# khimansusinha/Distributed-sorting-with-fault-tolerance

Measured on AMD Instinct MI355X. Metric: sorted keys/sec (int32, 2^30 keys), higher is better.
Workload: dtype int32; 1 GPU; C2-style single-GPU sort of 1073741824 uniform int32 keys (BASELINE metric size); tile 8192 keys, 0 merge passes; keys=1073741824, parallelism=1 GPU

## Files before the change

### distributed-sorting-with-fault-tolerance_amd/csrc/dsort_sub.h

```cpp
#pragma once
#include <hip/hip_runtime.h>
#include <stdint.h>

#include "dsort_bucket.h"

namespace dsort {
namespace sb {

constexpr int SB_T = 256;
constexpr int SB_MAXS = 1024;
constexpr int SB_SLOTB = 10;
constexpr int SB_SLOTS = 1 << SB_SLOTB;
#ifndef DSORT_SUB_TOTALS
#define DSORT_SUB_TOTALS 1
#endif
constexpr int SB_ST = 4;
template <typename T> constexpr int SB_KPT = sizeof(T) == 4 ? 16 : 8;
template <typename T> constexpr int SB_SUB = SB_T * SB_KPT<T>;
template <typename T> constexpr int SB_CH = SB_ST * SB_SUB<T>;

struct BInfo {
    uint64_t start;
    uint64_t soff;
    uint32_t len;
// ... 375 lines not shown
            aoff = off;
            v = 0;
            np = 0;
        }
        if (piece == 0 && np == 0 && v == 0) {
            ca = c + 1;
            aoff = 0;
        }
    }
    if (np) {
        f(ca, aoff, c1, v);
        ++nt;
    }
    return nt;
}
__device__ __forceinline__ uint2 tile_piece(const uint32_t *counts, int SS, uint32_t base, uint32_t c, uint32_t c0,
                                            uint32_t nch, uint32_t j0, uint32_t j1, uint32_t valid, uint32_t flags) {
    const uint32_t *pc = counts + (uint64_t)c * (SS + 1);
    const uint32_t lo = base + pc[j0] + (c == c0 ? flags >> 8 : 0u);
    return make_uint2(lo, nch == 1 ? lo + valid : base + pc[j1]);
}

#ifdef DSORT_STAMPS
__device__ unsigned long long g_sbstamps[(1u << 18) * 8];
#endif
template <bool LOCAL>
__global__ void __launch_bounds__(SB_MAXS, 8) sb_scan_kernel(const BInfo *__restrict__ bi, int SS,
                                                          const uint32_t *__restrict__ counts,
                                                          uint32_t *__restrict__ offs, int tile, int align,
                                                          uint32_t mis, uint32_t cpad, void *__restrict__ tiles,
                                                          uint32_t *__restrict__ ntiles, Ovf *__restrict__ ovf,
                                                          uint32_t *__restrict__ novf, uint32_t trec,
                                                          const Chunk *__restrict__ ch, uint2 *__restrict__ pieces,
                                                          uint32_t PS, uint32_t tcap, const uint32_t *__restrict__ stot) {
    __shared__ uint32_t wsum[SB_MAXS / 64];
    __shared__ uint32_t ss[SB_MAXS + 1];
    __shared__ uint16_t nxt[SB_MAXS];
    __shared__ uint16_t chain[SB_MAXS];
    __shared__ uint16_t tix[SB_MAXS];
    __shared__ uint32_t nchain, tbase;
#ifdef DSORT_SCAN_STAMPS
    uint64_t sc_acc[8] = {}, sc_t0 = __builtin_amdgcn_s_memtime();
#define SCST(k)                                            \
    do {                                                   \
        const uint64_t t1_ = __builtin_amdgcn_s_memtime(); \
        sc_acc[k] += t1_ - sc_t0;                          \
        sc_t0 = t1_;                                       \
    } while (0)
#else
#define SCST(k) \
    do {        \
    } while (0)
#endif
    const BInfo b = bi[blockIdx.x];
    const int j = threadIdx.x;
    const int ns = (int)b.nsub;
    const int full = tile;
    if (LOCAL) tile -= (int)(cpad * (b.c1 - b.c0));
    auto cnt = [&](uint32_t c) -> uint32_t {
        if constexpr (LOCAL) {
            const uint32_t *pc = counts + (uint64_t)c * (SS + 1);
            return pc[j + 1] - pc[j];
        } else {
            return counts[(uint64_t)c * SS + j];
        }
    };
    uint32_t tot = 0;
    if (LOCAL && stot) {
        if (j < ns) tot = stot[(uint64_t)blockIdx.x * SS + j];
    } else if constexpr (LOCAL) {
        uint32_t a = 0;
        if (j < ns) {
#ifndef DSORT_SCAN_SUM_U
#define DSORT_SCAN_SUM_U 16
#endif
#pragma unroll DSORT_SCAN_SUM_U
            for (uint32_t c = b.c0; c < b.c1; ++c) a += counts[(uint64_t)c * (SS + 1) + j + 1];
            ss[j + 1] = a;
        }
        __syncthreads();
        if (j < ns) tot = a - (j ? ss[j] : 0u);
    } else if (j < ns) {
#pragma unroll 8
        for (uint32_t c = b.c0; c < b.c1; ++c) tot += cnt(c);
    }
    uint32_t all;
// ... 491 lines not shown
```

### distributed-sorting-with-fault-tolerance_amd/csrc/dsort_wave.hip

```cpp
#include <hip/hip_runtime.h>

#include <stdint.h>

#include <algorithm>
#include <climits>
#include <ctime>
#include <sched.h>
#include <unistd.h>
#include <csignal>
#include <cstdlib>
#include <cstring>
#include <string>
#include <type_traits>
#include <vector>

#include "dsort_bucket.h"
#include "dsort_internal.h"
#include "dsort_tx.h"

#include <rocprofiler-sdk-roctx/roctx.h>
#include "dsort_part.h"
#include "dsort_sub.h"

namespace dsort {
// ... 977 lines not shown
                klo = gt.j0 > 0 ? sp[gt.j0 - 1].k : bk::Comp<T>::key_of(bs[gt.b - 1]);
                khi = gt.j1 < gt.nsub ? sp[gt.j1 - 1].k : bk::Comp<T>::key_of(bs[gt.b]);
            }
            if (jj < jh && jj + 1 < nspl) hint = sp[jj].k == sp[jj + 1].k;
            hint = __ballot(hint) != 0;
        }
        if (!late && known) {
            klo = gt.j0 > 0 ? sp[gt.j0 - 1].k : bk::Comp<T>::key_of(bs[gt.b - 1]);
            khi = gt.j1 < gt.nsub ? sp[gt.j1 - 1].k : bk::Comp<T>::key_of(bs[gt.b]);
#ifndef DSORT_ONEKEY_TILES
#define DSORT_ONEKEY_TILES 1
#endif
            if (DSORT_ONEKEY_TILES && sizeof(T) == 8 && klo == khi) {
                T *o = out + base;
                for (int i = (int)threadIdx.x; i < valid; i += (int)blockDim.x) o[i] = klo;
                return;
            }
        }
        if (!late) {
            if (jj < jh && jj + 1 < nspl) hint = sp[jj].k == sp[jj + 1].k;
            hint = __ballot(hint) != 0;
            gather_tile<T, W>(ga, pe, gt, in, s32 + 128, s32 + 96, x, threadIdx.x);
        }
    } else {
        j = toff + blockIdx.x;
        if (!load_tile<T, false, W>(in, n, tiles, ntiles, ga, j, nullptr, nullptr, x, base, valid)) return;
        if (valid == 0) return;
    }
    STAMP(1);
    if (!bin_sort_tile<T, W>(x, valid, s, cw, out + base, hint, known, klo, khi, threadIdx.x) && threadIdx.x == 0)
        fb[atomicAdd(nfb, 1u)] = j;
}

template <typename T, bool GATHER, int W>
__global__ void __launch_bounds__(64 * W, WG<T>::OCC) block_sort_w_kernel(
    const T *in, T *out, uint64_t n, const uint4 *tiles, const uint32_t *ntiles, sb::Gather ga,
    const uint32_t *fb, const uint32_t *nfb) {
    constexpr int TILE = TILE_W<W>, N = KPC<T>;
    using V = typename V16<T>::type;
    __shared__ __attribute__((aligned(16))) T s[TILE + WK];
    const int t = lane_id();
    const int w = __builtin_amdgcn_readfirstlane(threadIdx.x >> 6);
    const T c[6] = {lane_side<T>(0), lane_side<T>(1), lane_side<T>(2), lane_side<T>(3), lane_side<T>(4),
                    lane_side<T>(5)};
    const uint32_t nj = *nfb;
#pragma unroll 1
    for (uint32_t i = blockIdx.x; i < nj; i += gridDim.x) {
    if (i != blockIdx.x) __syncthreads();
    T x[R];
    uint64_t base;
    int valid;
    const uint32_t j = fb[i];
    if (!load_tile<T, GATHER, W>(in, n, tiles, ntiles, ga, j, reinterpret_cast<uint32_t *>(s) + 64,
                              reinterpret_cast<uint32_t *>(s), x, base, valid))
        return;
    if (GATHER) __syncthreads();
    sort_wave(x, c);
    {
        if (w & 1) {
            V *dst = reinterpret_cast<V *>(s + w * WK + WK - R * (t + 1));
#pragma unroll
            for (int q = 0; q < R / N; ++q) {
                T rv[N];
#pragma unroll
                for (int j = 0; j < N; ++j) rv[j] = x[R - 1 - (N * q + j)];
                dst[q] = V16<T>::make(rv);
            }
        } else {
            V *dst = reinterpret_cast<V *>(s + w * WK + t * R);
#pragma unroll
            for (int q = 0; q < R / N; ++q) dst[q] = V16<T>::make(x + N * q);
        }
    }
    __syncthreads();
    const int lo = out_lo(t);
#pragma unroll 1
    for (int r = WK; r < TILE; r <<= 1) {
        const int wpp = (2 * r) / WK;
        const int j = w / wpp, o = w % wpp;
        const int ps = j * 2 * r;
        const bool last = 2 * r == TILE;
        WinD win{ps, r, r, o * WK, 0, WK, !last && (j & 1)};
        merge_window_desc(s, win, x, c[0], c[1], c[2], c[3]);
        __syncthreads();
        if (last) {
            const int lim = valid - o * WK;
            win.cnt = lim < WK ? lim : WK;
            if (lim > 0) store_window_desc<false>(out + base, win, ps, lo, x);
        } else {
            store_window_desc<true>(s, win, ps, lo, x);
            __syncthreads();
        }
    }
    }
}

template <typename T, int LOGF, bool REG>
__global__ void __launch_bounds__(64 * WG<T>::MWAVES, WG<T>::OCC) mergew_kernel(
    const T *__restrict__ in, T *__restrict__ out, PassDesc pd, int tnom, const uint32_t *__restrict__ splits) {
    constexpr int WAVES = WG<T>::MWAVES, THREADS = 64 * WAVES, TILE = MTILE_OF<T>;
    constexpr int N = KPC<T>, LN = LKPC<T>;
    using V = typename V16<T>::type;
    constexpr int F = 1 << LOGF;
    constexpr int MAXWIN = (WAVES + F / 2 + WAVES - 1) / WAVES;
    static_assert(WAVES * MAXWIN <= 64, "window table: one lane per window");
    __shared__ __attribute__((aligned(16))) T s[TILE + WK];
    __shared__ int soff[F + 1];
    __shared__ int cpre[F + 1];
    __shared__ int4 sinfo[F];
    __shared__ int64_t sa0[F];
    __shared__ uint64_t s_out;
    __shared__ int4 wtab_a[LOGF][WAVES * MAXWIN];
    __shared__ int4 wtab_b[LOGF][WAVES * MAXWIN];
    const int t = lane_id();
    const int w = __builtin_amdgcn_readfirstlane(threadIdx.x >> 6);
    const uint64_t j = blockIdx.x;
    STAMP(0);
    RSTAMP(13);
    TileInfo ti;
    const GroupK *g = tile_info<REG>(pd, j, tnom, ti);
    if (threadIdx.x < 64) {
        const int i = t & (F - 1);
        uint64_t rs, rl;
        run_range<REG>(pd, ti, g, i, rs, rl);
        const uint32_t s0 = splits[j * F + i];
        const uint32_t s1 = ti.jr + 1 == ti.ntg ? (uint32_t)rl : splits[(j + 1) * F + i];
        const int len = (int)(s1 - s0);
// ... 156 lines not shown
    std::vector<int> out;
    const int bits = ceil_log2(runs);
    if (bits == 0) return out;
    const int cap = max_logf(opt, 4, WG<T>::MAXLOGF);
    const int P = (bits + cap - 1) / cap;
    for (int p = 0; p < P; ++p) out.push_back(bits / P + (p < bits % P ? 1 : 0));
    return out;
}

static void stage_range(const dsort_ctx *ctx, int i) {
    if (ctx->nested) return;
    switch (i) {
        case 9: roctxRangePushA("dsort:histogram"); break;
        case 11: roctxRangePushA("dsort:scatter"); break;
        case 13: roctxRangePushA("dsort:second-level"); break;
        case 7: roctxRangePushA("dsort:tile-sort"); break;
        case 10: case 12: case 14: case 8: roctxRangePop(); break;
        default: break;
    }
}
static int stage_event(dsort_ctx *ctx, hipStream_t s, bool timed, int i) {
    if (timed) stage_range(ctx, i);
    if (!timed || !ctx->ev_ok) return DSORT_OK;
    if (i == 1 || i == 7 || i == 8 || i == 13 || i == 14) i += ctx->ev_off;
    DSORT_HIP(ctx, hipEventRecord(ctx->ev[i], s));
    ctx->ev_mask |= 1u << i;
    return DSORT_OK;
}
static int tile_sort_event(dsort_ctx *ctx, hipStream_t s, bool timed, int which) {
    return stage_event(ctx, s, timed, 7 + which);
}

constexpr uint32_t kFallbackWgs = 512;
template <typename T, bool GATHER, int W>
static int tile_sort_begin(dsort_ctx *ctx, const T *in, T *out, uint64_t n, const uint4 *tiles, const uint32_t *ntiles,
                           const sb::Gather &ga, uint32_t grid, uint32_t cap, hipStream_t s) {
    int rc = ensure(ctx, &ctx->tfb, &ctx->tfb_bytes, ((size_t)cap + 1) * 4, "tile fallback list");
    if (rc) return rc;
    uint32_t *fb = static_cast<uint32_t *>(ctx->tfb), *nfb = fb + cap;
    DSORT_HIP(ctx, hipMemsetAsync(nfb, 0, 4, s));
    if (grid)
        hipLaunchKernelGGL((bin_sort_kernel<T, GATHER, W>), dim3(grid), dim3(64 * W), 0, s, in, out, n, tiles, ntiles, ga, fb,
                           nfb, 0u);
    DSORT_HIP(ctx, hipGetLastError());
    return DSORT_OK;
}
template <typename T, bool GATHER, int W>
static int tile_sort_more(dsort_ctx *ctx, const T *in, T *out, uint64_t n, const uint4 *tiles, const uint32_t *ntiles,
                          const sb::Gather &ga, uint32_t toff, uint32_t grid, uint32_t cap, hipStream_t s) {
    uint32_t *fb = static_cast<uint32_t *>(ctx->tfb), *nfb = fb + cap;
    if (grid)
        hipLaunchKernelGGL((bin_sort_kernel<T, GATHER, W>), dim3(grid), dim3(64 * W), 0, s, in, out, n, tiles, ntiles, ga, fb,
                           nfb, toff);
    DSORT_HIP(ctx, hipGetLastError());
    return DSORT_OK;
}
template <typename T, bool GATHER, int W>
static int tile_sort_end(dsort_ctx *ctx, const T *in, T *out, uint64_t n, const uint4 *tiles, const uint32_t *ntiles,
                         const sb::Gather &ga, uint32_t tiles_total, uint32_t cap, hipStream_t s) {
    const uint32_t *fb = static_cast<const uint32_t *>(ctx->tfb), *nfb = fb + cap;
    const uint32_t fgrid = tiles_total < kFallbackWgs ? tiles_total : kFallbackWgs;
    if (fgrid)
        hipLaunchKernelGGL((block_sort_w_kernel<T, GATHER, W>), dim3(fgrid), dim3(64 * W), 0, s, in, out, n, tiles, ntiles,
                           ga, fb, nfb);
    DSORT_HIP(ctx, hipGetLastError());
    return DSORT_OK;
}
template <typename T, bool GATHER, int W>
static int tile_sort_w(dsort_ctx *ctx, const T *in, T *out, uint64_t n, const uint4 *tiles, const uint32_t *ntiles,
                       const sb::Gather &ga, uint32_t grid, hipStream_t s) {
    int rc = tile_sort_begin<T, GATHER, W>(ctx, in, out, n, tiles, ntiles, ga, grid, grid, s);
    if (rc) return rc;
    return tile_sort_end<T, GATHER, W>(ctx, in, out, n, tiles, ntiles, ga, grid, grid, s);
}
template <typename T, typename F>
static int with_tile_waves(dsort_ctx *ctx, int tile, F &&f) {
    if (tile == TILE_OF<T>) return f(std::integral_constant<int, WG<T>::WAVES>{});
    if constexpr (sizeof(T) == 4)
        if (tile == TILE_W<16>) return f(std::integral_constant<int, 16>{});
    return set_err(ctx, DSORT_EINVAL, "tile sort: no kernel for this tile size");
}
template <typename T, bool GATHER>
static int tile_sort(dsort_ctx *ctx, const T *in, T *out, uint64_t n, const uint4 *tiles, const uint32_t *ntiles,
                     const sb::Gather &ga, uint32_t grid, hipStream_t s, bool timed, int tile = TILE_OF<T>) {
    int rc = tile_sort_event(ctx, s, timed, 0);
    if (rc) return rc;
    if (grid) {
        rc = with_tile_waves<T>(ctx, tile, [&](auto w) {
            return tile_sort_w<T, GATHER, decltype(w)::value>(ctx, in, out, n, tiles, ntiles, ga, grid, s);
        });
        if (rc) return rc;
    }
    return tile_sort_event(ctx, s, timed, 1);
}

template <typename T, bool REG>
static int launch_pass_w(dsort_ctx *ctx, const T *src, T *dst, const PassDesc &pd, int logf,
                         uint64_t ntiles, hipStream_t s, bool timed) {
    int rc = ensure(ctx, &ctx->splits, &ctx->splits_bytes,
                    (size_t)(ntiles + 1) * (size_t)(1 << logf) * sizeof(uint32_t), "split vectors");
    if (rc) return rc;
    uint32_t *sp = static_cast<uint32_t *>(ctx->splits);
    constexpr int TN = MTNOM_OF<T>;
    hipLaunchKernelGGL((partk_kernel<T, REG>), dim3((unsigned)ceil_div(ntiles, 4)), dim3(256), 0, s, src, pd,
                       TN, MSLACK_OF<T>, sp, ntiles);
    DSORT_HIP(ctx, hipGetLastError());
    const bool kt = timed && ctx->ev_ok && ctx->kev_used + 2 <= dsort_ctx::kMaxKev;
    if (kt) DSORT_HIP(ctx, hipEventRecord(ctx->kev[ctx->kev_used], s));
    const dim3 grid((unsigned)ntiles), block(64 * WG<T>::MWAVES);
    switch (logf) {
        case 1: hipLaunchKernelGGL((mergew_kernel<T, 1, REG>), grid, block, 0, s, src, dst, pd, TN, sp); break;
        case 2: hipLaunchKernelGGL((mergew_kernel<T, 2, REG>), grid, block, 0, s, src, dst, pd, TN, sp); break;
        case 3: hipLaunchKernelGGL((mergew_kernel<T, 3, REG>), grid, block, 0, s, src, dst, pd, TN, sp); break;
        case 4: hipLaunchKernelGGL((mergew_kernel<T, 4, REG>), grid, block, 0, s, src, dst, pd, TN, sp); break;
        case 5:
            if constexpr (WG<T>::MAXLOGF >= 5) {
                hipLaunchKernelGGL((mergew_kernel<T, 5, REG>), grid, block, 0, s, src, dst, pd, TN, sp);
                break;
            }
            return set_err(ctx, DSORT_EINVAL, "bad pass fan-in");
        default: return set_err(ctx, DSORT_EINVAL, "bad pass fan-in");
    }
    DSORT_HIP(ctx, hipGetLastError());
    if (kt) {
        DSORT_HIP(ctx, hipEventRecord(ctx->kev[ctx->kev_used + 1], s));
        ctx->kev_used += 2;
// ... 271 lines not shown
    DSORT_HIP(ctx, hipMemcpyAsync(stl, hst, B * sizeof(bk::TileRef) + 16, hipMemcpyHostToDevice, ctx->side));
    DSORT_HIP(ctx, hipMemsetAsync(num, 0, 8, ctx->side));
    if (nfill)
        DSORT_HIP(ctx, hipMemcpyAsync(a + o_fill, hf, nfill * sizeof(FillSeg<T>), hipMemcpyHostToDevice, ctx->side));
    DSORT_HIP(ctx, hipEventRecord(ctx->side_ev, ctx->side));
    DSORT_HIP(ctx, hipStreamWaitEvent(s, ctx->side_ev, 0));
    uint64_t npure = 0;
    for (int b = 0; b < B; ++b) npure += pure[b] ? hb[b + 1] - hb[b] : 0;
    ctx->stats.tile_sort_keys = n - npure;
    if (nfill) {
        const unsigned gx = (unsigned)std::min<uint64_t>(ceil_div(maxfill, 256 * FILL_U * (16 / sizeof(T))), 1024);
        hipLaunchKernelGGL(fill_segments_kernel<T>, dim3(gx, nfill), dim3(256), 0, s, d_keys,
                           reinterpret_cast<const FillSeg<T> *>(a + o_fill));
        DSORT_HIP(ctx, hipGetLastError());
    }
    for (int b = 0; b < B && !pure_done && !pm;) {
        if (!pure[b]) {
            ++b;
            continue;
        }
        int e = b;
        while (e < B && pure[e]) ++e;
        if (hb[e] > hb[b])
            DSORT_HIP(ctx, hipMemcpyAsync(d_keys + hb[b], src + hb[b], (hb[e] - hb[b]) * sizeof(T),
                                          hipMemcpyDeviceToDevice, s));
        b = e;
    }
    if (nsmp) {
        hipLaunchKernelGGL(sb_sample_kernel<T>, dim3((unsigned)B), dim3(SB_T), 0, s, src, dbi, dch, smp, cmp);
        DSORT_HIP(ctx, hipGetLastError());
        const uint4 *stl4 = reinterpret_cast<const uint4 *>(stl);
        const uint32_t *pnst = reinterpret_cast<const uint32_t *>(stl + B);
        if constexpr (sizeof(T) == 8) {
            rc = tile_sort<int64_t, false>(ctx, smp, srt, nsmp, stl4, pnst, sb::Gather{}, nst, s, false);
            if (rc) return rc;
            hipLaunchKernelGGL(sb_rank_kernel, dim3((unsigned)B), dim3(SB_T), 0, s, smp, srt, dbi, cmp);
        }
        rc = tile_sort<int64_t, false>(ctx, cmp, cmp, nsmp, stl4, pnst, sb::Gather{}, nst, s, false);
        if (rc) return rc;
        hipLaunchKernelGGL(sb_splitter_kernel<T>, dim3((unsigned)B), dim3(SB_MAXS), 0, s, cmp, smp, dbi, dch, os, SS, spl,
                           rng, sfn, stot);
        DSORT_HIP(ctx, hipGetLastError());
    } else if (stot) {
        DSORT_HIP(ctx, hipMemsetAsync(stot, 0, (size_t)B * SS * 4, s));
    }
    const uint32_t mis = (uint32_t)((reinterpret_cast<uintptr_t>(d_keys) / sizeof(T)) & (ALIGN - 1));
    uint32_t *hn = reinterpret_cast<uint32_t *>(h + h_num);
    if (local) {
        if (nch) {
            if ((rc = stage_event(ctx, s, timed, 13))) return rc;
            hipLaunchKernelGGL(sb_local_kernel<T>, dim3((unsigned)nch), dim3(SB_LT<T>), 0, s, src, dch, dbi, SS, spl, rng,
                               sfn, cnt, ctx->bk_hot, stot);
            DSORT_HIP(ctx, hipGetLastError());
            if ((rc = stage_event(ctx, s, timed, 14))) return rc;
        }
#ifndef DSORT_PIECES_SCAN_MINB
#define DSORT_PIECES_SCAN_MINB 256
#endif
        const bool pieces_in_scan = B >= DSORT_PIECES_SCAN_MINB;
        hipLaunchKernelGGL(sb_scan_kernel<true>, dim3((unsigned)B), dim3(SB_MAXS), 0, s, dbi, SS, cnt, nullptr, TILE, 1,
                           0u, (uint32_t)(2 * (ALIGN - 1)), tt, num, ovf, num + 1, (uint32_t)tmax,
                           static_cast<const Chunk *>(dch), pieces_in_scan ? pcs : nullptr, PS, (uint32_t)tcap, stot);
        DSORT_HIP(ctx, hipGetLastError());
        const Gather ga{static_cast<const GTile *>(tt), dch, dbi, cnt, pcs, PS, SS, spl, bspl, B,
                        (uint32_t)std::max<uint64_t>(tcap, 1)};
#ifndef DSORT_PIECES_EARLY
#define DSORT_PIECES_EARLY 1
#endif
        const bool pieces_early = DSORT_PIECES_EARLY && !pieces_in_scan && pcs && tcap > 0;
        if (pieces_early) {
            hipLaunchKernelGGL(sb_pieces_kernel, dim3((unsigned)ceil_div(tcap, 4)), dim3(256), 0, s,
                               static_cast<const GTile *>(tt), num, static_cast<const Chunk *>(dch), cnt, SS, pcs, PS,
                               (uint32_t)tcap);
            DSORT_HIP(ctx, hipGetLastError());
        }
        DSORT_HIP(ctx, hipMemcpyAsync(hn, num, 8, hipMemcpyDeviceToHost, s));
        DSORT_HIP(ctx, hipEventRecord(ctx->sub_ev, s));
#ifndef DSORT_TILE_EARLY
#define DSORT_TILE_EARLY 1
#endif
        const uint64_t ebound = (n - npure) / (uint64_t)TILE;
        const uint32_t early = DSORT_TILE_EARLY && (pieces_in_scan || pieces_early) && ctx->opt.kill_after_pass != 1
                                   ? (uint32_t)std::min<uint64_t>(ebound, tcap)
                                   : 0u;
        if (early) {
            if ((rc = tile_sort_event(ctx, s, timed, 0))) return rc;
            rc = with_tile_waves<T>(ctx, TILE, [&](auto w) {
                return tile_sort_begin<T, true, decltype(w)::value>(ctx, src, d_keys, n, nullptr, num, ga, early,
                                                                    (uint32_t)tcap, s);
            });
            if (rc) return rc;
        }
        if (int rc_ = sync_event(ctx, ctx->sub_ev, "tile count")) return rc_;
        const uint32_t ntiles = hn[0], novf = hn[1];
        if (ntiles > tmax || ntiles > tcap) {
            if (early)
                if (int rc_ = sync_stream(ctx, s, "early tile sort")) return rc_;
            ctx->stats.sub_scatter_fallback = 1;
            return sub_sort<T>(ctx, src, d_keys, n, hb, B, m, s, timed, false, pure, pure_done, bspl, true, pm,
                               fill_keys);
        }
        if (ntiles && !pieces_in_scan && !pieces_early) {
            hipLaunchKernelGGL(sb_pieces_kernel, dim3((unsigned)ceil_div(ntiles, 4)), dim3(256), 0, s,
                               static_cast<const GTile *>(tt), num, static_cast<const Chunk *>(dch), cnt, SS, pcs, PS,
                               (uint32_t)tcap);
            DSORT_HIP(ctx, hipGetLastError());
        }
        fault_point(ctx, s, 1);
        ctx->stats.merge_passes = 0;
        if (early) {
            rc = with_tile_waves<T>(ctx, TILE, [&](auto w) {
                constexpr int W = decltype(w)::value;
                int r = tile_sort_more<T, true, W>(ctx, src, d_keys, n, nullptr, num, ga, early,
                                                   ntiles > early ? ntiles - early : 0u, (uint32_t)tcap, s);
                return r ? r : tile_sort_end<T, true, W>(ctx, src, d_keys, n, nullptr, num, ga, ntiles, (uint32_t)tcap, s);
            });
            if (rc) return rc;
            if ((rc = tile_sort_event(ctx, s, timed, 1))) return rc;
        } else if (ntiles) {
            rc = tile_sort<T, true>(ctx, src, d_keys, n, nullptr, num, ga, ntiles, s, timed, TILE);
            if (rc) return rc;
        }
        if ((rc = stage_event(ctx, s, timed, 1))) return rc;
        fault_point(ctx, s, 2);
        if (novf) {
            rc = merge_split_subbuckets<T>(ctx, ovf, novf, static_cast<const GTile *>(tt), d_keys, s);
            if (rc) return rc;
        }
        if (timed && ctx->ev_ok) {
            DSORT_HIP(ctx, hipEventRecord(ctx->ev[ctx->ev_done], s));
            ctx->ev_mask |= 1u << ctx->ev_done;
        }
        return DSORT_OK;
    }
    if (nch) {
        if ((rc = stage_event(ctx, s, timed, 13))) return rc;
        hipLaunchKernelGGL(sb_hist_kernel<T>, dim3((unsigned)nch), dim3(SB_T), 0, s, src, dch, dbi, SS, spl, rng,
                           sfn, cnt);
        DSORT_HIP(ctx, hipGetLastError());
    }
    hipLaunchKernelGGL(sb_scan_kernel<false>, dim3((unsigned)B), dim3(SB_MAXS), 0, s, dbi, SS, cnt, offs, TILE,
                       (int)ALIGN, mis, 0u, tt, num, ovf, num + 1, (uint32_t)tmax, nullptr, nullptr, 0u, 0u, nullptr);
    DSORT_HIP(ctx, hipGetLastError());
    DSORT_HIP(ctx, hipMemcpyAsync(hn, num, 8, hipMemcpyDeviceToHost, s));
    DSORT_HIP(ctx, hipEventRecord(ctx->sub_ev, s));
    if (nch) {
        hipLaunchKernelGGL(sb_scatter_kernel<T>, dim3((unsigned)nch), dim3(SB_T), 0, s, src, d_keys, dch,
                           (uint32_t)nch, dbi, SS, spl, rng, sfn, offs);
        DSORT_HIP(ctx, hipGetLastError());
        if ((rc = stage_event(ctx, s, timed, 14))) return rc;
    }
    if (int rc_ = sync_event(ctx, ctx->sub_ev, "tile count")) return rc_;
    const uint32_t ntiles = hn[0], novf = hn[1];
    if (ntiles > tmax || novf > nsubs) return set_err(ctx, DSORT_EHIP, "sub-bucket packing overflow");
    fault_point(ctx, s, 1);
    ctx->stats.merge_passes = 0;
    if (ntiles) {
        rc = tile_sort<T, false>(ctx, d_keys, d_keys, n, static_cast<const uint4 *>(tt), num, Gather{}, ntiles, s,
                                 timed, TILE);
        if (rc) return rc;
    }
    if (timed && ctx->ev_ok) {
        DSORT_HIP(ctx, hipEventRecord(ctx->ev[1], s));
        ctx->ev_mask |= 2u;
    }
    fault_point(ctx, s, 2);
    if (novf) {
        std::vector<Ovf> ov(novf);
        DSORT_HIP(ctx, hipMemcpyAsync(ov.data(), ovf, novf * sizeof(Ovf), hipMemcpyDeviceToHost, s));
        if (int rc_ = sync_stream(ctx, s, "sort stream")) return rc_;
        uint64_t mx = 0;
        for (const Ovf &o : ov) mx = o.len > mx ? o.len : mx;
        if (int rc_ = ensure(ctx, &ctx->stmp, &ctx->stmp_bytes, mx * sizeof(T) + 16, "oversized sub-bucket merge"))
            return rc_;
        T *tmp = static_cast<T *>(ctx->stmp);
// ... 144 lines not shown
            if (!Comp<T>::ADAPT && RB && hm->hot)
                hipLaunchKernelGGL((bucket_scatter_lines_kernel<T, false, false, true>), dim3((unsigned)L.G), dim3(BK_T), 0,
                                   s, d_in, n, L.spl, L.map, B, BP, L.subs, L.offs, part_out, direct, ioff, L.ids);
            else
                hipLaunchKernelGGL((bucket_scatter_lines_kernel<T, false, false>), dim3((unsigned)L.G), dim3(BK_T), 0, s,
                                   d_in, n, L.spl, L.map, B, BP, L.subs, L.offs, part_out, direct, ioff, L.ids);
        }
    }
    if constexpr (BkIds<T>::ON)
        if (!RB || ids)
            hipLaunchKernelGGL((bucket_scatter_lines_kernel<T, true>), dim3((unsigned)L.G), dim3(BK_T), 0, s, d_in, n,
                               L.spl, L.map, B, BP, L.subs, L.offs, part_out, direct, ioff, L.ids);
    DSORT_HIP(ctx, hipGetLastError());
    if ((rc = stage_event(ctx, s, timed, 12))) return rc;
    fault_point(ctx, s, 0);
    if (int rc_ = sync_event(ctx, ctx->bucket_ev, "bucket starts")) return rc_;
    if (hb[B] != n) return set_err(ctx, DSORT_EHIP, "bucket partition lost keys");
    ctx->stats.first_level_map = !Comp<T>::ADAPT && !ad ? (RB && hm->r2s ? 3 : 0) : hm->mode == 0 ? 1 : 2;
    return DSORT_OK;
}

static int bucketed_stats_start(dsort_ctx *ctx, uint64_t n, int tile, hipStream_t s, bool timed) {
    ctx->bk_hot = nullptr;
    ctx->stats = fresh_stats();
    ctx->stats.keys_in = ctx->stats.keys_out = n;
    ctx->stats.tile_sort_keys = n;
    ctx->stats.tile_keys = tile;
    ctx->ev_mask = 0;
    ctx->kev_used = 0;
    ctx->last_stream = s;
    return stage_event(ctx, s, timed, 0);
}

template <typename T>
static int bucket_sort(dsort_ctx *ctx, const T *d_in, T *d_keys, size_t n, hipStream_t s, bool timed, int B) {
    using namespace bk;
    using C = typename Comp<T>::C;
    constexpr int TILE = TILE_OF<T>;
    constexpr uint64_t ALIGN = KPC<T>;
    const int os = bucket_os(ctx);
    const uint32_t S = (uint32_t)B * (uint32_t)os;
    BkLayout<T> L;
    int rc = bk_layout<T>(ctx, n, B, (size_t)S * (sizeof(T) == 8 ? 24 : sizeof(C)), L);
    if (rc) return rc;
    const int BP = L.BP;
    C *smp = reinterpret_cast<C *>(L.smp);
    C *spl = L.spl;
    TileRef *tt = L.tt;
    uint32_t *ntl = L.ntl;
    const uint64_t tmax = L.tmax;
    rc = ensure(ctx, &ctx->scratch, &ctx->scratch_bytes, n * sizeof(T) + 16, "sort scratch");
    if (rc) return rc;
    T *scratch = static_cast<T *>(ctx->scratch);
    int64_t *pk = reinterpret_cast<int64_t *>(smp), *psrt = pk + S, *pcmp = pk + 2 * (size_t)S;
    ++ctx->nested;
    if constexpr (std::is_same<T, int32_t>::value) {
        hipLaunchKernelGGL(bucket_sample_kernel<T>, dim3(ceil_div(S, 256)), dim3(256), 0, s, d_in, (uint64_t)n, smp, S);
        rc = hipGetLastError() == hipSuccess ? sort_device<int64_t>(ctx, smp, smp, S, s, false)
                                             : set_err(ctx, DSORT_EHIP, "bucket_sample_kernel launch");
    } else {
        hipLaunchKernelGGL(pair_sample_keys_kernel, dim3(ceil_div(S, 256)), dim3(256), 0, s, d_in, (uint64_t)n, pk, S);
        rc = sort_device<int64_t>(ctx, pk, psrt, S, s, false);
        if (!rc) {
            hipLaunchKernelGGL(pair_rank_kernel, dim3(ceil_div(S, 256)), dim3(256), 0, s, pk, psrt, S, pcmp);
            rc = sort_device<int64_t>(ctx, pcmp, pcmp, S, s, false);
        }
    }
    --ctx->nested;
    if (rc) return rc;
    if ((rc = bucketed_stats_start(ctx, n, TILE, s, timed))) return rc;
    if constexpr (std::is_same<T, int32_t>::value) {
        hipLaunchKernelGGL(bucket_splitter_kernel<int32_t>, dim3(1), dim3(BK_MAXB), 0, s, smp, B, BP, os, spl);
    } else {
        hipLaunchKernelGGL(pair_splitter_kernel, dim3(1), dim3(BK_MAXB), 0, s, pcmp, pk, (uint64_t)n, S, B, BP, os,
                           spl);
    }
    T *part_out = scratch;
    T *direct = sub_keys<T>(ctx) && (const void *)d_in != (const void *)d_keys && n < (1ull << 31) ? d_keys : nullptr;
    uint64_t *hb;
    C *hspl;
    rc = first_level<T>(ctx, d_in, n, 0, part_out, direct, L, sub_keys<T>(ctx) ? 0u : (uint32_t)TILE, s, timed, hb,
                        hspl);
    if (rc) return rc;
    if (const uint64_t m = sub_keys<T>(ctx)) {
        std::vector<uint8_t> pure((size_t)B, 0);
        for (int b = 1; b + 1 < B; ++b) pure[b] = Comp<T>::key_of(hspl[b - 1]) == Comp<T>::key_of(hspl[b]);
        std::vector<T> fk;
        if (direct && DSORT_DROP_PURE) {
            fk.assign((size_t)B, T(0));
            for (int b = 1; b + 1 < B; ++b)
                if (pure[b]) fk[b] = Comp<T>::key_of(hspl[b]);
        }
        return sub_sort<T>(ctx, part_out, d_keys, n, hb, B, m, s, timed, ctx->opt.sub_gather != 0, pure.data(),
                           direct != nullptr, spl, false, nullptr, fk.empty() ? nullptr : fk.data());
    }
    std::vector<std::vector<uint64_t>> runs(B);
    uint64_t maxruns = 1;
    for (int b = 0; b < B; ++b) {
        const uint64_t len = hb[b + 1] - hb[b], h = bucket_head(hb[b], len, ALIGN);
        if (h) runs[b].push_back(h);
        for (uint64_t o = h; o < len; o += TILE) runs[b].push_back(len - o < (uint64_t)TILE ? len - o : TILE);
        maxruns = runs[b].size() > maxruns ? runs[b].size() : maxruns;
    }
    const std::vector<int> pbits = plan_passes<T>(ctx->opt, maxruns);
// ... 369 lines not shown
static int wave_sort(dsort_ctx *ctx, const T *d_in, T *d_keys, size_t n, hipStream_t s, bool timed) {
    constexpr int TILE = TILE_OF<T>;
    ctx->stats = fresh_stats();
    ctx->stats.keys_in = n;
    ctx->stats.keys_out = n;
    ctx->stats.tile_keys = TILE;
    ctx->ev_mask = 0;
    ctx->kev_used = 0;
    ctx->last_stream = s;
    if (n < 2) {
        if (n == 1 && d_in != d_keys)
            DSORT_HIP(ctx, hipMemcpyAsync(d_keys, d_in, sizeof(T), hipMemcpyDeviceToDevice, s));
        return DSORT_OK;
    }
    if (const int B = bucket_count(ctx, n)) return bucket_sort<T>(ctx, d_in, d_keys, n, s, timed, B);
    const uint64_t tiles = ceil_div(n, TILE);
    const std::vector<int> plan = plan_passes<T>(ctx->opt, tiles);
    const int passes = (int)plan.size();
    ctx->stats.merge_passes = passes;
    T *scratch = nullptr;
    if (passes > 0) {
        void **sb = ctx->nested ? &ctx->scratch2 : &ctx->scratch;
        size_t *sbb = ctx->nested ? &ctx->scratch2_bytes : &ctx->scratch_bytes;
        int rc = ensure(ctx, sb, sbb, n * sizeof(T), "sort scratch");
        if (rc) return rc;
        scratch = static_cast<T *>(*sb);
    }
    T *bufs[2] = {d_keys, scratch};
    int cur = (passes % 2 == 0) ? 0 : 1;
    if (timed && ctx->ev_ok) {
        DSORT_HIP(ctx, hipEventRecord(ctx->ev[0], s));
        ctx->ev_mask |= 1u;
    }
    int rc = tile_sort<T, false>(ctx, d_in, bufs[cur], n, nullptr, nullptr, sb::Gather{}, (uint32_t)tiles, s, timed);
    if (rc) return rc;
    if (timed && ctx->ev_ok) {
        DSORT_HIP(ctx, hipEventRecord(ctx->ev[1], s));
        ctx->ev_mask |= 2u;
    }
    fault_point(ctx, s, 0);
    constexpr uint64_t MTN = MTNOM_OF<T>;
    uint64_t Rr = TILE;
    for (int p = 0; p < passes; ++p) {
        PassDesc pd{(uint64_t)n, Rr, 1 << plan[p], 0, nullptr};
        const uint64_t gsize = Rr << plan[p];
        const uint64_t ngroups = ceil_div(n, gsize);
        const uint64_t tpg = ceil_div(gsize, MTN);
        const uint64_t mtiles = (ngroups - 1) * tpg + ceil_div(n - (ngroups - 1) * gsize, MTN);
        int rc = launch_pass_w<T, true>(ctx, bufs[cur], bufs[cur ^ 1], pd, plan[p], mtiles, s, timed);
        if (rc) return rc;
        Rr <<= plan[p];
        cur ^= 1;
        fault_point(ctx, s, 1 + p);
    }
    if (timed && ctx->ev_ok) {
        DSORT_HIP(ctx, hipEventRecord(ctx->ev[2], s));
        ctx->ev_mask |= 4u;
    }
    return DSORT_OK;
}

template <typename T>
static int wave_merge(dsort_ctx *ctx, const T *d_in, const size_t *lens, int k, T *d_out, hipStream_t s,
                      bool keep_stats) {
    constexpr int MAXF = 1 << WG<T>::MAXLOGF;
    if (!keep_stats) {
        ctx->stats = fresh_stats();
// ... 198 lines not shown
```

Baseline: 143.9 billion keys/s.

## Fuse sample tile sort fallback, select splitters from sorted runs, fold counter reset

Adds a sample_tile_sort kernel that runs bin sort and falls back in-block to the bitonic path, replacing the two-kernel fallback scheme for nested int64 sample sorts. When the sample fits in 2-16 tiles, it skips the merge passes and picks splitters straight from the sorted runs with a new wave-parallel bucket_select_kernel. The scan kernel now zeroes the tile fallback counter itself, which drops a memset. The aim is fewer launches and less serialized work in the sampling and splitter phase, at the cost of a more involved selection kernel with tricky iteration logic.

```diff
diff --git a/distributed-sorting-with-fault-tolerance_amd/csrc/dsort_sub.h b/distributed-sorting-with-fault-tolerance_amd/csrc/dsort_sub.h
--- a/distributed-sorting-with-fault-tolerance_amd/csrc/dsort_sub.h
+++ b/distributed-sorting-with-fault-tolerance_amd/csrc/dsort_sub.h
@@ -431,7 +431,8 @@
                                                           uint32_t *__restrict__ ntiles, Ovf *__restrict__ ovf,
                                                           uint32_t *__restrict__ novf, uint32_t trec,
                                                           const Chunk *__restrict__ ch, uint2 *__restrict__ pieces,
-                                                          uint32_t PS, uint32_t tcap, const uint32_t *__restrict__ stot) {
+                                                          uint32_t PS, uint32_t tcap, const uint32_t *__restrict__ stot,
+                                                          uint32_t *__restrict__ zero) {
     __shared__ uint32_t wsum[SB_MAXS / 64];
     __shared__ uint32_t ss[SB_MAXS + 1];
     __shared__ uint16_t nxt[SB_MAXS];
@@ -451,6 +452,7 @@
     do {        \
     } while (0)
 #endif
+    if (zero && blockIdx.x == 0 && threadIdx.x == 0) *zero = 0;
     const BInfo b = bi[blockIdx.x];
     const int j = threadIdx.x;
     const int ns = (int)b.nsub;
diff --git a/distributed-sorting-with-fault-tolerance_amd/csrc/dsort_wave.hip b/distributed-sorting-with-fault-tolerance_amd/csrc/dsort_wave.hip
--- a/distributed-sorting-with-fault-tolerance_amd/csrc/dsort_wave.hip
+++ b/distributed-sorting-with-fault-tolerance_amd/csrc/dsort_wave.hip
@@ -1033,15 +1033,57 @@
         fb[atomicAdd(nfb, 1u)] = j;
 }
 
+template <typename T, int W>
+__device__ __forceinline__ void bitonic_tile(T (&x)[R], const T (&c)[6], T *s, T *out, int valid) {
+    constexpr int TILE = TILE_W<W>, N = KPC<T>;
+    using V = typename V16<T>::type;
+    const int t = lane_id();
+    const int w = __builtin_amdgcn_readfirstlane(threadIdx.x >> 6);
+    sort_wave(x, c);
+    {
+        if (w & 1) {
+            V *dst = reinterpret_cast<V *>(s + w * WK + WK - R * (t + 1));
+#pragma unroll
+            for (int q = 0; q < R / N; ++q) {
+                T rv[N];
+#pragma unroll
+                for (int j = 0; j < N; ++j) rv[j] = x[R - 1 - (N * q + j)];
+                dst[q] = V16<T>::make(rv);
+            }
+        } else {
+            V *dst = reinterpret_cast<V *>(s + w * WK + t * R);
+#pragma unroll
+            for (int q = 0; q < R / N; ++q) dst[q] = V16<T>::make(x + N * q);
+        }
+    }
+    __syncthreads();
+    const int lo = out_lo(t);
+#pragma unroll 1
+    for (int r = WK; r < TILE; r <<= 1) {
+        const int wpp = (2 * r) / WK;
+        const int j = w / wpp, o = w % wpp;
+        const int ps = j * 2 * r;
+        const bool last = 2 * r == TILE;
+        WinD win{ps, r, r, o * WK, 0, WK, !last && (j & 1)};
+        merge_window_desc(s, win, x, c[0], c[1], c[2], c[3]);
+        __syncthreads();
+        if (last) {
+            const int lim = valid - o * WK;
+            win.cnt = lim < WK ? lim : WK;
+            if (lim > 0) store_window_desc<false>(out, win, ps, lo, x);
+        } else {
+            store_window_desc<true>(s, win, ps, lo, x);
+            __syncthreads();
+        }
+    }
+}
+
 template <typename T, bool GATHER, int W>
 __global__ void __launch_bounds__(64 * W, WG<T>::OCC) block_sort_w_kernel(
     const T *in, T *out, uint64_t n, const uint4 *tiles, const uint32_t *ntiles, sb::Gather ga,
     const uint32_t *fb, const uint32_t *nfb) {
-    constexpr int TILE = TILE_W<W>, N = KPC<T>;
-    using V = typename V16<T>::type;
+    constexpr int TILE = TILE_W<W>;
     __shared__ __attribute__((aligned(16))) T s[TILE + WK];
-    const int t = lane_id();
-    const int w = __builtin_amdgcn_readfirstlane(threadIdx.x >> 6);
     const T c[6] = {lane_side<T>(0), lane_side<T>(1), lane_side<T>(2), lane_side<T>(3), lane_side<T>(4),
                     lane_side<T>(5)};
     const uint32_t nj = *nfb;
@@ -1056,44 +1098,30 @@
                               reinterpret_cast<uint32_t *>(s), x, base, valid))
         return;
     if (GATHER) __syncthreads();
-    sort_wave(x, c);
-    {
-        if (w & 1) {
-            V *dst = reinterpret_cast<V *>(s + w * WK + WK - R * (t + 1));
-#pragma unroll
-            for (int q = 0; q < R / N; ++q) {
-                T rv[N];
-#pragma unroll
-                for (int j = 0; j < N; ++j) rv[j] = x[R - 1 - (N * q + j)];
-                dst[q] = V16<T>::make(rv);
-            }
-        } else {
-            V *dst = reinterpret_cast<V *>(s + w * WK + t * R);
-#pragma unroll
-            for (int q = 0; q < R / N; ++q) dst[q] = V16<T>::make(x + N * q);
-        }
-    }
-    __syncthreads();
-    const int lo = out_lo(t);
-#pragma unroll 1
-    for (int r = WK; r < TILE; r <<= 1) {
-        const int wpp = (2 * r) / WK;
-        const int j = w / wpp, o = w % wpp;
-        const int ps = j * 2 * r;
-        const bool last = 2 * r == TILE;
-        WinD win{ps, r, r, o * WK, 0, WK, !last && (j & 1)};
-        merge_window_desc(s, win, x, c[0], c[1], c[2], c[3]);
-        __syncthreads();
-        if (last) {
-            const int lim = valid - o * WK;
-            win.cnt = lim < WK ? lim : WK;
-            if (lim > 0) store_window_desc<false>(out + base, win, ps, lo, x);
-        } else {
-            store_window_desc<true>(s, win, ps, lo, x);
-            __syncthreads();
-        }
-    }
-    }
+    bitonic_tile<T, W>(x, c, s, out + base, valid);
+    }
+}
+
+#ifndef DSORT_SAMPLE_SORT_SELF
+#define DSORT_SAMPLE_SORT_SELF 1
+#endif
+template <typename T, int W>
+__global__ void __launch_bounds__(64 * W, WG<T>::OCC) sample_tile_sort_kernel(const T *in, T *out, uint64_t n,
+                                                                             const uint4 *tiles,
+                                                                             const uint32_t *ntiles) {
+    constexpr int TILE = TILE_W<W>;
+    __shared__ __attribute__((aligned(16))) T s[TILE + WK];
+    __shared__ __attribute__((aligned(16))) uint32_t cw[BIN_NB<W> / 2];
+    reinterpret_cast<uint4 *>(cw)[threadIdx.x] = make_uint4(0u, 0u, 0u, 0u);
+    T x[R];
+    uint64_t base;
+    int valid;
+    if (!load_tile<T, false, W>(in, n, tiles, ntiles, sb::Gather{}, blockIdx.x, nullptr, nullptr, x, base, valid)) return;
+    if (valid == 0) return;
+    if (bin_sort_tile<T, W>(x, valid, s, cw, out + base, false, false, T(0), T(0), threadIdx.x)) return;
+    const T c[6] = {lane_side<T>(0), lane_side<T>(1), lane_side<T>(2), lane_side<T>(3), lane_side<T>(4),
+                    lane_side<T>(5)};
+    bitonic_tile<T, W>(x, c, s, out + base, valid);
 }
 
 template <typename T, int LOGF, bool REG>
@@ -1316,13 +1344,19 @@
 }
 
 constexpr uint32_t kFallbackWgs = 512;
+static int tile_fallback_counter(dsort_ctx *ctx, uint32_t cap, uint32_t **nfb) {
+    int rc = ensure(ctx, &ctx->tfb, &ctx->tfb_bytes, ((size_t)cap + 1) * 4, "tile fallback list");
+    if (rc) return rc;
+    *nfb = static_cast<uint32_t *>(ctx->tfb) + cap;
+    return DSORT_OK;
+}
 template <typename T, bool GATHER, int W>
 static int tile_sort_begin(dsort_ctx *ctx, const T *in, T *out, uint64_t n, const uint4 *tiles, const uint32_t *ntiles,
-                           const sb::Gather &ga, uint32_t grid, uint32_t cap, hipStream_t s) {
+                           const sb::Gather &ga, uint32_t grid, uint32_t cap, hipStream_t s, bool zeroed = false) {
     int rc = ensure(ctx, &ctx->tfb, &ctx->tfb_bytes, ((size_t)cap + 1) * 4, "tile fallback list");
     if (rc) return rc;
     uint32_t *fb = static_cast<uint32_t *>(ctx->tfb), *nfb = fb + cap;
-    DSORT_HIP(ctx, hipMemsetAsync(nfb, 0, 4, s));
+    if (!zeroed) DSORT_HIP(ctx, hipMemsetAsync(nfb, 0, 4, s));
     if (grid)
         hipLaunchKernelGGL((bin_sort_kernel<T, GATHER, W>), dim3(grid), dim3(64 * W), 0, s, in, out, n, tiles, ntiles, ga, fb,
                            nfb, 0u);
@@ -1376,6 +1410,14 @@
         if (rc) return rc;
     }
     return tile_sort_event(ctx, s, timed, 1);
+}
+static int sample_tile_sort(dsort_ctx *ctx, const int64_t *in, int64_t *out, uint64_t n, const uint4 *tiles,
+                            const uint32_t *ntiles, uint32_t grid, hipStream_t s) {
+    if (!DSORT_SAMPLE_SORT_SELF) return tile_sort<int64_t, false>(ctx, in, out, n, tiles, ntiles, sb::Gather{}, grid, s, false);
+    constexpr int W = WG<int64_t>::WAVES;
+    if (grid) hipLaunchKernelGGL((sample_tile_sort_kernel<int64_t, W>), dim3(grid), dim3(64 * W), 0, s, in, out, n, tiles, ntiles);
+    DSORT_HIP(ctx, hipGetLastError());
+    return DSORT_OK;
 }
 
 template <typename T, bool REG>
@@ -1713,11 +1755,11 @@
         const uint4 *stl4 = reinterpret_cast<const uint4 *>(stl);
         const uint32_t *pnst = reinterpret_cast<const uint32_t *>(stl + B);
         if constexpr (sizeof(T) == 8) {
-            rc = tile_sort<int64_t, false>(ctx, smp, srt, nsmp, stl4, pnst, sb::Gather{}, nst, s, false);
+            rc = sample_tile_sort(ctx, smp, srt, nsmp, stl4, pnst, nst, s);
             if (rc) return rc;
             hipLaunchKernelGGL(sb_rank_kernel, dim3((unsigned)B), dim3(SB_T), 0, s, smp, srt, dbi, cmp);
         }
-        rc = tile_sort<int64_t, false>(ctx, cmp, cmp, nsmp, stl4, pnst, sb::Gather{}, nst, s, false);
+        rc = sample_tile_sort(ctx, cmp, cmp, nsmp, stl4, pnst, nst, s);
         if (rc) return rc;
         hipLaunchKernelGGL(sb_splitter_kernel<T>, dim3((unsigned)B), dim3(SB_MAXS), 0, s, cmp, smp, dbi, dch, os, SS, spl,
                            rng, sfn, stot);
@@ -1739,24 +1781,10 @@
 #define DSORT_PIECES_SCAN_MINB 256
 #endif
         const bool pieces_in_scan = B >= DSORT_PIECES_SCAN_MINB;
-        hipLaunchKernelGGL(sb_scan_kernel<true>, dim3((unsigned)B), dim3(SB_MAXS), 0, s, dbi, SS, cnt, nullptr, TILE, 1,
-                           0u, (uint32_t)(2 * (ALIGN - 1)), tt, num, ovf, num + 1, (uint32_t)tmax,
-                           static_cast<const Chunk *>(dch), pieces_in_scan ? pcs : nullptr, PS, (uint32_t)tcap, stot);
-        DSORT_HIP(ctx, hipGetLastError());
-        const Gather ga{static_cast<const GTile *>(tt), dch, dbi, cnt, pcs, PS, SS, spl, bspl, B,
-                        (uint32_t)std::max<uint64_t>(tcap, 1)};
 #ifndef DSORT_PIECES_EARLY
 #define DSORT_PIECES_EARLY 1
 #endif
         const bool pieces_early = DSORT_PIECES_EARLY && !pieces_in_scan && pcs && tcap > 0;
-        if (pieces_early) {
-            hipLaunchKernelGGL(sb_pieces_kernel, dim3((unsigned)ceil_div(tcap, 4)), dim3(256), 0, s,
-                               static_cast<const GTile *>(tt), num, static_cast<const Chunk *>(dch), cnt, SS, pcs, PS,
-                               (uint32_t)tcap);
-            DSORT_HIP(ctx, hipGetLastError());
-        }
-        DSORT_HIP(ctx, hipMemcpyAsync(hn, num, 8, hipMemcpyDeviceToHost, s));
-        DSORT_HIP(ctx, hipEventRecord(ctx->sub_ev, s));
 #ifndef DSORT_TILE_EARLY
 #define DSORT_TILE_EARLY 1
 #endif
@@ -1764,11 +1792,32 @@
         const uint32_t early = DSORT_TILE_EARLY && (pieces_in_scan || pieces_early) && ctx->opt.kill_after_pass != 1
                                    ? (uint32_t)std::min<uint64_t>(ebound, tcap)
                                    : 0u;
+#ifndef DSORT_SCAN_ZEROES_TFB
+#define DSORT_SCAN_ZEROES_TFB 1
+#endif
+        uint32_t *nfb0 = nullptr;
+        if (DSORT_SCAN_ZEROES_TFB && early)
+            if ((rc = tile_fallback_counter(ctx, (uint32_t)tcap, &nfb0))) return rc;
+        hipLaunchKernelGGL(sb_scan_kernel<true>, dim3((unsigned)B), dim3(SB_MAXS), 0, s, dbi, SS, cnt, nullptr, TILE, 1,
+                           0u, (uint32_t)(2 * (ALIGN - 1)), tt, num, ovf, num + 1, (uint32_t)tmax,
+                           static_cast<const Chunk *>(dch), pieces_in_scan ? pcs : nullptr, PS, (uint32_t)tcap, stot,
+                           nfb0);
+        DSORT_HIP(ctx, hipGetLastError());
+        const Gather ga{static_cast<const GTile *>(tt), dch, dbi, cnt, pcs, PS, SS, spl, bspl, B,
+                        (uint32_t)std::max<uint64_t>(tcap, 1)};
+        if (pieces_early) {
+            hipLaunchKernelGGL(sb_pieces_kernel, dim3((unsigned)ceil_div(tcap, 4)), dim3(256), 0, s,
+                               static_cast<const GTile *>(tt), num, static_cast<const Chunk *>(dch), cnt, SS, pcs, PS,
+                               (uint32_t)tcap);
+            DSORT_HIP(ctx, hipGetLastError());
+        }
+        DSORT_HIP(ctx, hipMemcpyAsync(hn, num, 8, hipMemcpyDeviceToHost, s));
+        DSORT_HIP(ctx, hipEventRecord(ctx->sub_ev, s));
         if (early) {
             if ((rc = tile_sort_event(ctx, s, timed, 0))) return rc;
             rc = with_tile_waves<T>(ctx, TILE, [&](auto w) {
                 return tile_sort_begin<T, true, decltype(w)::value>(ctx, src, d_keys, n, nullptr, num, ga, early,
-                                                                    (uint32_t)tcap, s);
+                                                                    (uint32_t)tcap, s, nfb0 != nullptr);
             });
             if (rc) return rc;
         }
@@ -1821,7 +1870,8 @@
         DSORT_HIP(ctx, hipGetLastError());
     }
     hipLaunchKernelGGL(sb_scan_kernel<false>, dim3((unsigned)B), dim3(SB_MAXS), 0, s, dbi, SS, cnt, offs, TILE,
-                       (int)ALIGN, mis, 0u, tt, num, ovf, num + 1, (uint32_t)tmax, nullptr, nullptr, 0u, 0u, nullptr);
+                       (int)ALIGN, mis, 0u, tt, num, ovf, num + 1, (uint32_t)tmax, nullptr, nullptr, 0u, 0u, nullptr,
+                       nullptr);
     DSORT_HIP(ctx, hipGetLastError());
     DSORT_HIP(ctx, hipMemcpyAsync(hn, num, 8, hipMemcpyDeviceToHost, s));
     DSORT_HIP(ctx, hipEventRecord(ctx->sub_ev, s));
@@ -2032,6 +2082,120 @@
     return stage_event(ctx, s, timed, 0);
 }
 
+#ifndef DSORT_SPLIT_SELECT
+#define DSORT_SPLIT_SELECT 1
+#endif
+__global__ void __launch_bounds__(256) bucket_select_kernel(const int64_t *__restrict__ runs, uint32_t S, uint32_t run,
+                                                            int F, int B, int BP, int os,
+                                                            const int64_t *__restrict__ keys, uint64_t n,
+                                                            void *__restrict__ spl) {
+    int64_t *spl32 = static_cast<int64_t *>(spl);
+    bk::Pair *spl64 = static_cast<bk::Pair *>(spl);
+    if (blockIdx.x == 0)
+        for (int b = B - 1 + (int)threadIdx.x; b < BP; b += 256) {
+            if (keys) spl64[b] = bk::Comp<int64_t>::inf();
+            else spl32[b] = bk::Comp<int32_t>::inf();
+        }
+    const int lane = threadIdx.x & 63;
+    const int b = (int)blockIdx.x * 4 + (int)(threadIdx.x >> 6);
+    if (b >= B - 1) return;
+    const int C = 64 / F;
+    const int i = lane & (F - 1), c = lane / F;
+    const uint64_t rs = (uint64_t)i * run < S ? (uint64_t)i * run : S, rl = S - rs < run ? S - rs : run;
+    const int64_t *A = runs + rs;
+    const uint64_t d = (uint64_t)(b + 1) * (uint64_t)os;
+    int64_t lo = wave_min(rl ? A[0] : key_max<int64_t>());
+    int64_t hi = wave_max(rl ? A[rl - 1] : key_min<int64_t>());
+    uint64_t ilo = 0, ihi = rl, nlo = 0, nhi = S;
+    int mode = 0;
+#pragma unroll 1
+    for (int it = 0; it < 4096 && nhi - nlo > 64 && lo != hi; ++it) {
+        int64_t cand;
+        const double m = (double)(nhi - nlo);
+        const double spread = fmax(24.0, 3.0 * sqrt(m));
+        const double r = C == 1 ? 0.0 : -spread + 2.0 * spread * (double)c / (double)(C - 1);
+        if (mode == 0) {
+            cand = key_at(lo, hi, ((double)d + r - (double)nlo) / m);
+        } else {
+            const uint64_t packed = wave_max(((ihi - ilo) << 6) | (uint64_t)(63 - i));
+            const int rr = 63 - (int)(packed & 63);
+            double frac = mode == 1 ? ((double)d + r - (double)nlo) / m : (double)(c + 1) / (double)(C + 1);
+            frac = frac < 0.0 ? 0.0 : (frac > 1.0 ? 1.0 : frac);
+            int64_t mine = key_max<int64_t>();
+            if (i == rr) {
+                const uint64_t range = ihi - ilo;
+                uint64_t pos = ilo + (uint64_t)(frac * (double)range);
+                pos = pos >= ihi ? ihi - 1 : pos;
+                mine = A[pos];
+            }
+            cand = __shfl(mine, c * F + rr);
+            cand = cand < hi ? cand : hi - 1;
+        }
+        const uint64_t u = upper_bound_interp(A, ilo, ihi, cand, lo, hi, runs + S);
+        uint64_t tot = u;
+        for (int o = 1; o < F; o <<= 1) tot += __shfl_xor(tot, o);
+        const unsigned long long mask = __ballot(tot >= d);
+        const int cs = mask ? (int)((__ffsll((long long)mask) - 1) / F) : C;
+        const uint64_t ub_cs = __shfl(u, (cs < C ? cs : 0) * F + i);
+        const uint64_t ub_pr = __shfl(u, (cs > 0 ? cs - 1 : 0) * F + i);
+        const uint64_t tot_cs = __shfl(tot, (cs < C ? cs : 0) * F);
+        const uint64_t tot_pr = __shfl(tot, (cs > 0 ? cs - 1 : 0) * F);
+        const int64_t cand_cs = __shfl(cand, (cs < C ? cs : 0) * F);
+        const int64_t cand_pr = __shfl(cand, (cs > 0 ? cs - 1 : 0) * F);
+        const uint64_t before = nhi - nlo;
+        if (cs < C) {
+            hi = cand_cs;
+            ihi = ub_cs;
+            nhi = tot_cs;
+        }
+        if (cs > 0) {
+            lo = cand_pr + 1;
+            ilo = ub_pr;
+            nlo = tot_pr;
+        }
+        if (mode != 0) {
+            lo = wave_min(ilo < ihi ? A[ilo] : key_max<int64_t>());
+            hi = wave_max(ilo < ihi ? A[ihi - 1] : key_min<int64_t>());
+        }
+        const bool halved = (nhi - nlo) * 2 <= before;
+        mode = halved ? (mode == 2 ? 1 : mode) : (mode == 0 ? 1 : 2);
+    }
+    int64_t x = key_max<int64_t>();
+    bool mine = false;
+    if (nhi - nlo > 64) {
+        x = lo;
+        mine = lane == 0;
+    } else {
+        uint32_t e = 0;
+        uint64_t at = 0;
+        bool have = false;
+        for (int q = 0; q < F; ++q) {
+            const uint32_t ql = (uint32_t)__shfl((int)(uint32_t)ilo, q), qn = (uint32_t)__shfl((int)(uint32_t)(ihi - ilo), q);
+            if ((uint32_t)lane >= e && (uint32_t)lane < e + qn) {
+                at = (uint64_t)q * run + ql + ((uint32_t)lane - e);
+                have = true;
+            }
+            e += qn;
+        }
+        have = have && at < S;
+        if (have) x = runs[at];
+        uint32_t rank = 0;
+        for (int k = 0; k < 64; ++k) {
+            const int64_t y = __shfl(x, k);
+            rank += (y < x || (y == x && k < lane)) ? 1u : 0u;
+        }
+        mine = have && rank == (uint32_t)(d - 1 - nlo);
+    }
+    if (mine) {
+        if (keys) {
+            const uint32_t g = (uint32_t)x;
+            spl64[b] = bk::Pair{keys[g], (uint32_t)bk::sample_pos(g, n, S), 0};
+        } else {
+            spl32[b] = x;
+        }
+    }
+}
+
 template <typename T>
 static int bucket_sort(dsort_ctx *ctx, const T *d_in, T *d_keys, size_t n, hipStream_t s, bool timed, int B) {
     using namespace bk;
@@ -2053,23 +2217,34 @@
     if (rc) return rc;
     T *scratch = static_cast<T *>(ctx->scratch);
     int64_t *pk = reinterpret_cast<int64_t *>(smp), *psrt = pk + S, *pcmp = pk + 2 * (size_t)S;
+    constexpr uint32_t STILE = TILE_OF<int64_t>;
+    const uint32_t stiles = (uint32_t)ceil_div(S, STILE);
+    const bool select = DSORT_SPLIT_SELECT && stiles >= 2 && stiles <= 16;
+    auto sort_composites = [&](int64_t *c) {
+        return select ? sample_tile_sort(ctx, c, c, S, nullptr, nullptr, stiles, s) : sort_device<int64_t>(ctx, c, c, S, s, false);
+    };
     ++ctx->nested;
     if constexpr (std::is_same<T, int32_t>::value) {
         hipLaunchKernelGGL(bucket_sample_kernel<T>, dim3(ceil_div(S, 256)), dim3(256), 0, s, d_in, (uint64_t)n, smp, S);
-        rc = hipGetLastError() == hipSuccess ? sort_device<int64_t>(ctx, smp, smp, S, s, false)
+        rc = hipGetLastError() == hipSuccess ? sort_composites(smp)
                                              : set_err(ctx, DSORT_EHIP, "bucket_sample_kernel launch");
     } else {
         hipLaunchKernelGGL(pair_sample_keys_kernel, dim3(ceil_div(S, 256)), dim3(256), 0, s, d_in, (uint64_t)n, pk, S);
         rc = sort_device<int64_t>(ctx, pk, psrt, S, s, false);
         if (!rc) {
             hipLaunchKernelGGL(pair_rank_kernel, dim3(ceil_div(S, 256)), dim3(256), 0, s, pk, psrt, S, pcmp);
-            rc = sort_device<int64_t>(ctx, pcmp, pcmp, S, s, false);
+            rc = sort_composites(pcmp);
         }
     }
     --ctx->nested;
     if (rc) return rc;
     if ((rc = bucketed_stats_start(ctx, n, TILE, s, timed))) return rc;
-    if constexpr (std::is_same<T, int32_t>::value) {
+    if (select) {
+        const bool w8 = sizeof(T) == 8;
+        hipLaunchKernelGGL(bucket_select_kernel, dim3((unsigned)ceil_div((uint64_t)B - 1, 4)), dim3(256), 0, s,
+                           w8 ? pcmp : reinterpret_cast<const int64_t *>(smp), S, STILE, 1 << ceil_log2(stiles), B, BP, os,
+                           w8 ? pk : nullptr, (uint64_t)n, static_cast<void *>(spl));
+    } else if constexpr (std::is_same<T, int32_t>::value) {
         hipLaunchKernelGGL(bucket_splitter_kernel<int32_t>, dim3(1), dim3(BK_MAXB), 0, s, smp, B, BP, os, spl);
     } else {
         hipLaunchKernelGGL(pair_splitter_kernel, dim3(1), dim3(BK_MAXB), 0, s, pcmp, pk, (uint64_t)n, S, B, BP, os,
@@ -2505,7 +2680,13 @@
         DSORT_HIP(ctx, hipEventRecord(ctx->ev[0], s));
         ctx->ev_mask |= 1u;
     }
-    int rc = tile_sort<T, false>(ctx, d_in, bufs[cur], n, nullptr, nullptr, sb::Gather{}, (uint32_t)tiles, s, timed);
+    int rc;
+    if constexpr (sizeof(T) == 8) {
+        rc = ctx->nested ? sample_tile_sort(ctx, d_in, bufs[cur], n, nullptr, nullptr, (uint32_t)tiles, s)
+                         : tile_sort<T, false>(ctx, d_in, bufs[cur], n, nullptr, nullptr, sb::Gather{}, (uint32_t)tiles, s, timed);
+    } else {
+        rc = tile_sort<T, false>(ctx, d_in, bufs[cur], n, nullptr, nullptr, sb::Gather{}, (uint32_t)tiles, s, timed);
+    }
     if (rc) return rc;
     if (timed && ctx->ev_ok) {
         DSORT_HIP(ctx, hipEventRecord(ctx->ev[1], s));
```

Result: no change. 143.7 billion keys/s (-0.1%).
